# aakhundov/tf-attend-infer-repeat

Measured on AMD Instinct MI355X. Metric: images/sec AIR train step, 50x50 multi-MNIST b=64 N=3, higher is better.
Workload: dtype bf16; 1 GPU; configs[1]: AIR train step, 50x50 canvas, 0-2 objects, batch 64/GPU, 3 steps, 256 LSTM, z=50 (training.py:100-122); global_batch=64, hipgraph=True, steps_per_graph_replay=20, graph_mode=one hipGraph replay = 20 train steps, parallelism=dp1, backward=reference, phase=single order

## Files before the change

tf-attend-infer-repeat_amd/csrc/air_sampler_common.h:

```cpp
#pragma once
#include "air_common.h"
#include <cstdio>
#include <atomic>
#include <type_traits>
#include <cstdlib>
#include <cstring>
#include <cmath>

namespace {

constexpr int THREADS = 256;

struct Tap { float w0, w1; int i0, i1; };

__device__ __forceinline__ Tap axis_tap(int j, int n_out, int n_in, float a, float b, float* t_out = nullptr) {
    const float step = 2.0f / (float)(n_out - 1);
    const float t = (n_out > 1) ? (-1.0f + step * (float)j) : -1.0f;
    const float xs = a * t + b;
    const float X = ((xs + 1.0f) * ((float)n_in - 1.001f)) / 2.0f;
    const float f0 = floorf(X);
    const float lim = (float)(n_in - 1);
    const float c0 = fminf(fmaxf(f0, 0.0f), lim);
    const float c1 = fminf(fmaxf(f0 + 1.0f, 0.0f), lim);
    Tap tp;
// ... 103 lines not shown
        R = R + sh_z[t] * wr;
    }
    return R;
}

__device__ __forceinline__ float compose_clip(float R, float& p1, float& p0) {
    const float r = fmaxf(fminf(R, 1.0f), 0.0f);
    p1 = r + AIR_EPS; p0 = (1.0f - r) + AIR_EPS;
    return r;
}
__device__ __forceinline__ float compose_dloss(float R, float x, float p1, float p0, float gsc) {
    const bool pass = (R <= 1.0f) && (fminf(R, 1.0f) >= 0.0f);
    return pass ? -gsc * (x / p1 - (1.0f - x) / p0) : 0.0f;
}

__device__ __forceinline__ float gauss_kl_term(float plv, float lv, float var, float pv, float mean, float pm) {
    const float d = mean - pm;
    return (((plv - lv) - 1.0f) + var / pv) + (d * d) / pv;
}

struct ComposeLds {
    float* red; float* z; int* act;
    float* kl; float* rec;
    Tap* tx; Tap* ty; float* win;
};
__device__ __forceinline__ ComposeLds compose_lds(float* base, int N, int C, int w) {
    ComposeLds L;
    L.red = base; L.z = base + 16; L.act = reinterpret_cast<int*>(base + 16 + MAX_STEPS);
    L.kl = base + 16 + 2 * MAX_STEPS; L.rec = base + 16 + 3 * MAX_STEPS;
    L.tx = reinterpret_cast<Tap*>(base + 16 + 7 * MAX_STEPS); L.ty = L.tx + (size_t)N * C;
    L.win = reinterpret_cast<float*>(L.ty + (size_t)N * C);
    return L;
}
template <int NWAVES>
__device__ __forceinline__ void compose_vae_kl(const float* ml_all, const float* dyn, int b, int B, int N, int Z, int lane, int wave,
                                               float* sh_kl) {
    for (int t = wave; t < N; t += NWAVES) {
        const float* ml = ml_all + ((size_t)t * B + b) * 2 * Z;
        const float pv = dyn[AIR_DYN_VAE_PV], pm = dyn[AIR_DYN_VAE_PM], plv = dyn[AIR_DYN_VAE_PLV];
        float klt = 0.0f;
        for (int j = lane; j < Z; j += 64) {
            const float lv = ml[Z + j];
            klt += gauss_kl_term(plv, lv, expf(lv), pv, ml[j], pm);
        }
        klt = air_wave_sum(klt);
        if (lane == 0) sh_kl[t] = 0.5f * klt;
    }
}
__device__ __forceinline__ void compose_fetch_records(const float* att, int b, int B, int N, int tid, const ComposeLds& L) {
    if (tid < N) {
        const float* at = att + ((size_t)tid * B + b) * AIR_ATT_STRIDE;
        const float zv = at[AIR_ATT_Z], mk = at[AIR_ATT_MASK], mp = at[AIR_ATT_MASK_PREV];
        const float kz = at[AIR_ATT_KL_Z], ks = at[AIR_ATT_KL_SCALE], kh = at[AIR_ATT_KL_SHIFT];
        L.z[tid] = zv;
        L.act[tid] = mk != 0.0f ? 1 : 0;
        L.rec[4 * tid] = mp; L.rec[4 * tid + 1] = kz; L.rec[4 * tid + 2] = ks; L.rec[4 * tid + 3] = kh;
    }
}
__device__ __forceinline__ void compose_running_loss(const ComposeLds& L, float* att, int b, int B, int N, float& loss, int& digits) {
    loss = 0.0f;
    digits = 0;
    for (int t = 0; t < N; ++t) {
        const bool mask = L.act[t] != 0;
        loss = loss + (L.rec[4 * t] != 0.0f ? L.rec[4 * t + 1] : 0.0f);
        loss = loss + (mask ? L.rec[4 * t + 2] : 0.0f);
        loss = loss + (mask ? L.rec[4 * t + 3] : 0.0f);
        loss = loss + (mask ? L.kl[t] : 0.0f);
        digits += mask ? 1 : 0;
        att[((size_t)t * B + b) * AIR_ATT_STRIDE + AIR_ATT_KL_VAE] = L.kl[t];
    }
}
constexpr int COMPOSE_XPRE = 4;
__device__ __forceinline__ bool compose_prefetch_image(const float* images, size_t base, int CC, int tid, float (&xs)[COMPOSE_XPRE]) {
    const bool xpre = CC <= COMPOSE_XPRE * CF_THREADS;
#pragma unroll
    for (int k = 0; k < COMPOSE_XPRE; ++k) { const int p = tid + k * CF_THREADS; xs[k] = images[base + ((xpre && p < CC) ? p : 0)]; }
    return xpre;
}
template <int OUT, bool G_LDS>
__device__ __forceinline__ float compose_pixels(const ComposeLds& L, const float* images, size_t base, const float (&xs)[COMPOSE_XPRE],
// ... 69 lines not shown
```

tf-attend-infer-repeat_amd/csrc/air_sampler_write_bwd.hip:

```cpp
#include "air_sampler_common.h"

AIR_STAMPS_READER(air_debug_stamps_wb)
#ifdef AIR_STAMPS
static __device__ unsigned long long air_stamps_wg[4096 * 8];
extern "C" int air_debug_stamps_wg(unsigned long long* out, int n) {
    return (int)hipMemcpyFromSymbol(out, HIP_SYMBOL(air_stamps_wg), sizeof(unsigned long long) * (n < 4096 * 8 ? n : 4096 * 8));
}
#define AIR_STAMP_WG(i) do { if (threadIdx.x == 0) air_stamps_wg[((blockIdx.y * gridDim.x + blockIdx.x) & 4095) * 8 + (i)] = wall_clock64(); } while (0)
#define AIR_STAMP_WG_T(i, t) do { if (threadIdx.x == (t)) air_stamps_wg[((blockIdx.y * gridDim.x + blockIdx.x) & 4095) * 8 + (i)] = wall_clock64(); } while (0)
#define AIR_STAMP_WG_ADD(i, t0) do { if (threadIdx.x == 0) air_stamps_wg[((blockIdx.y * gridDim.x + blockIdx.x) & 4095) * 8 + (i)] += wall_clock64() - (t0); } while (0)
#define AIR_STAMP_WG_SET(i, v) do { if (threadIdx.x == 0) air_stamps_wg[((blockIdx.y * gridDim.x + blockIdx.x) & 4095) * 8 + (i)] = (unsigned long long)(v); } while (0)
#define AIR_NOW() wall_clock64()
#else
#define AIR_STAMP_WG(i) do { } while (0)
#define AIR_STAMP_WG_T(i, t) do { } while (0)
#define AIR_STAMP_WG_ADD(i, t0) do { } while (0)
#define AIR_STAMP_WG_SET(i, v) do { } while (0)
#define AIR_NOW() 0ull
#endif

namespace {

typedef __attribute__((address_space(3))) float air_lds_float;
__device__ __forceinline__ void lds_fadd(float* p, float v) {
    asm volatile("ds_add_f32 %0, %1" :: "v"((unsigned)(size_t)(air_lds_float*)p), "v"(v) : "memory");
}

__global__ __launch_bounds__(THREADS) void transformer_bwd_kernel(
    const float* __restrict__ U, const float* __restrict__ theta, const float* __restrict__ d_out,
    float* __restrict__ d_U, float* __restrict__ d_theta, int Hi, int Wi, int Ho, int Wo, int lds_ordered)
{
    extern __shared__ __attribute__((aligned(16))) float smem[];
    const int b = blockIdx.x, tid = threadIdx.x, lane = tid & 63, wave = tid >> 6;
    const int NI = Hi * Wi, NO = Ho * Wo;
    float* sh_red = smem;
    float* sh_th = smem + 32;
    float* sh_U = smem + 40;
    float* sh_dU = sh_U + ((NI + 3) & ~3);
    const float* img = U + (size_t)b * NI;
    const float* g = d_out + (size_t)b * NO;
    if (tid < 6) sh_th[tid] = theta[(size_t)b * 6 + tid];
    for (int p = tid; p < NI; p += THREADS) { sh_U[p] = img[p]; sh_dU[p] = 0.0f; }
    __syncthreads();
    if (d_theta) {
        float s6[6] = {0.f, 0.f, 0.f, 0.f, 0.f, 0.f};
        for (int p = tid; p < NO; p += THREADS) {
            const GenTap t = generic_tap(sh_th, p / Wo, p % Wo, Hi, Wi, Ho, Wo);
            const float Ia = sh_U[t.y0 * Wi + t.x0], Ib = sh_U[t.y1 * Wi + t.x0];
            const float Ic = sh_U[t.y0 * Wi + t.x1], Id = sh_U[t.y1 * Wi + t.x1];
            generic_dtheta_pixel(t, g[p] * Ia, g[p] * Ib, g[p] * Ic, g[p] * Id, Hi, Wi, s6);
        }
// ... 483 lines not shown
template <bool ALLPH>
__device__ __forceinline__ bool wb_open(const air_write_bwd_t& a, WbCtx& k, float& win_pre, float (&g_pre)[8]) {
    if (a.fin_scalars && k.lin == (a.order ? (int)(gridDim.x * gridDim.y) - 1 : 0)) {
        batch_means<WB_THREADS>(a, k.sh_red, k.tid, LoadPlain{});
        __syncthreads();
    }
    AIR_STAMP(40);
    AIR_STAMP_WG(0);
    win_pre = k.tid < k.w * k.w ? k.v[k.tid] : 0.0f;
    if (ALLPH) stage_g_load<WB_THREADS>(k.gsrc, k.CC, k.tid, 0, g_pre);
    if (k.at[AIR_ATT_MASK] == 0.0f) {
        zero_item<WB_THREADS>(k.dgen, k.dgen16, k.dsx, k.w * k.w, k.tid);
        return false;
    }
    wb_item(k, k.at[AIR_ATT_S], k.at[AIR_ATT_X], k.at[AIR_ATT_Y], k.at[AIR_ATT_Z]);
    return true;
}

constexpr int WB_SIG = WB_THREADS - 64;
__device__ __forceinline__ int* fold_last_word(const WbCtx& k) { return reinterpret_cast<int*>(k.sh_red) + (WB_NW - 1) * 8 + 7; }
__device__ __forceinline__ int fold_signal(int32_t* arrive, int tid) {
    int ticket = -1;
    if (tid == WB_SIG) {
        asm volatile("s_waitcnt vmcnt(0)" ::: "memory");
        ticket = __hip_atomic_fetch_add((air_global_int*)arrive, 1, __ATOMIC_RELAXED, __HIP_MEMORY_SCOPE_AGENT);
    }
    return ticket;
}
__device__ __forceinline__ void fold_means(const air_write_bwd_t& a, int32_t* arrive, const WbCtx& k, bool last) {
    if (!last) return;
    batch_means<WB_THREADS>(a, k.sh_red, k.tid, LoadAgent{});
    if (k.tid == 0) store_agent(arrive, 0);
}
__device__ __forceinline__ bool fold_front(const air_write_bwd_t& a, const air_write_fwd_t& f, int32_t* arrive, WbCtx& k, bool owner,
                                           float& win_pre) {
    const int N = a.N, B = a.B, C = k.C, w = k.w, tid = k.tid, b = k.b;
    const ComposeLds L = compose_lds(k.sh_T, N, C, w);
    float* c_sig = L.win + (size_t)N * w * w;
    const size_t base = (size_t)b * k.CC;
    const float mask_own = k.at[AIR_ATT_MASK];
    wb_item(k, k.at[AIR_ATT_S], k.at[AIR_ATT_X], k.at[AIR_ATT_Y], k.at[AIR_ATT_Z]);
    constexpr int WPRE = 4;
    float xs[COMPOSE_XPRE], wpre[WPRE];
    const bool xpre = compose_prefetch_image(f.images, base, k.CC, tid, xs);
#pragma unroll
    for (int q = 0; q < WPRE; ++q) {
        const int it = tid + q * WB_THREADS;
        wpre[q] = compose_window_at(a.vrec, b, B, w, it < N * w * w ? it : 0);
    }
    if (owner) compose_vae_kl<WB_NW>(f.ml, f.dyn, b, B, N, f.Z, k.lane, k.wave, L.kl);
    compose_stage_taps(a.att, b, B, N, C, w, tid, WB_THREADS, L.tx, L.ty);
#pragma unroll
    for (int q = 0; q < WPRE; ++q) { const int it = tid + q * WB_THREADS; if (it < N * w * w) L.win[it] = wpre[q]; }
    compose_stage_windows(a.vrec, b, B, N, w, tid + WPRE * WB_THREADS, WB_THREADS, L.win);
    compose_fetch_records(a.att, b, B, N, tid, L);
    __syncthreads();
    if (!owner && mask_own == 0.0f) {
        zero_item<WB_THREADS>(k.dgen, k.dgen16, k.dsx, w * w, tid);
        return false;
    }
    if (owner && tid == 0) {
        float loss;
        int digits;
        compose_running_loss(L, f.att, b, B, N, loss, digits);
        f.run_loss[b] = loss;
        c_sig[0] = loss;
        c_sig[1] = __builtin_bit_cast(float, digits);
    }
    float acc = compose_pixels<2, true>(L, f.images, base, xs, xpre, N, C, w, f.dyn[AIR_DYN_GRAD_SCALE], tid, owner,
                                        f.recon, f.d_recon, k.sh_g);
    if (owner) {
        acc = air_block_sum_n<WB_NW>(acc, L.red);
        const float rl = -acc;
        if (tid == 0) f.rec_loss[b] = rl;
        if (tid == WB_SIG) {
            store_agent(f.loss_item + b, c_sig[0] + rl);
            store_agent(f.run_digits + b, __builtin_bit_cast(int, c_sig[1]));
        }
    }
    AIR_STAMP_WG(7);
    if (mask_own == 0.0f) {
        zero_item<WB_THREADS>(k.dgen, k.dgen16, k.dsx, w * w, tid);
        const int ticket = fold_signal(arrive, tid);
        int* sh_last = fold_last_word(k);
        if (tid == WB_SIG) *sh_last = ticket == a.B - 1 ? 1 : 0;
        __syncthreads();
        fold_means(a, arrive, k, *sh_last != 0);
        return false;
    }
    win_pre = tid < w * w ? L.win[(size_t)k.t * w * w + tid] : 0.0f;
    return true;
}

template <bool ALLPH, int PH0, int PH1>
__device__ __forceinline__ void stage_terms(const WbCtx& k) {
    const int C = k.C, di = WB_THREADS / C, dj = WB_THREADS % C;
    int i = k.tid / C, j = k.tid % C;
    for (int p = k.tid; p < k.CC; p += WB_THREADS) {
        const Tap tx = k.sh_tx[j], ty = k.sh_ty[i];
        const float gp = k.z * (ALLPH ? k.sh_g[p] : k.gsrc[p]);
        const int4 ci = k.sh_ci[j], ri = k.sh_ri[i];
#pragma unroll
        for (int ph = PH0; ph < PH1; ++ph)
            k.sh_T[(ALLPH ? ph * k.CCp : 0) + wb_term_pos(ci, ri, i, j, C, ph)] = wb_tap_weight(tx, ty, ph) * gp;
        i += di; j += dj;
        if (j >= C) { j -= C; ++i; }
    }
}
template <bool ALLPH, int PH0, int PH1, bool THETA>
__device__ __forceinline__ void carried_terms(const WbCtx& k, WbGrad& G) {
    const int C = k.C, w = k.w;
    const int RPP = WB_THREADS / C, bj = k.tid % C, bi0 = k.tid / C;
    if (bi0 >= RPP) return;
// ... 318 lines not shown
}
template <bool ALLPH>
__device__ __forceinline__ bool carried_slot_short(const WbCtx& k, const WbSlot& s) {
    bool short_s = true;
    if (s.is_slot) {
#pragma unroll
        for (int ph = 0; ph < 4; ++ph) { int st, n; slot_run<ALLPH>(k, ph, s.sp, s.sq, st, n); short_s = short_s && n <= WB_CHUNK_MIN; }
    }
    return short_s;
}
template <bool ALLPH, int PH0, int PH1>
__device__ __forceinline__ void carried_slot(const WbCtx& k, const WbSlot& s, float& P_s, float& corr_s, float& Q_s, bool short_s, bool& have_s,
                                             float& acc) {
    if (!s.is_slot) return;
#pragma unroll
    for (int ph = PH0; ph < PH1; ++ph) {
        int start, n;
        slot_run<ALLPH>(k, ph, s.sp, s.sq, start, n);
        n = max(n, 0);
        if (short_s) { acc = stream_add(acc, k.sh_T, start, n); continue; }
        const int cs = wb_chunk_len(n);
        for (int k0 = 0; k0 < n; k0 += cs) {
            if (have_s) corr_s += Q_s - P_s;
            float c = 0.0f, q = P_s;
            stream_add2(c, q, k.sh_T, start + k0, min(cs, n - k0));
            Q_s = q;
            P_s += c;
            have_s = true;
        }
        acc = Q_s + corr_s;
    }
}

template <bool FOLD>
__device__ __forceinline__ void write_bwd_graph_allph_body(const air_write_bwd_t& a, int seq_flags, const air_write_fwd_t* fp,
                                                           int32_t* arrive) {
    extern __shared__ __attribute__((aligned(16))) float smem[];
    const bool lds_ordered = seq_flags & 1, ring_ok = seq_flags & 2;
    WbCtx k = wb_ctx<true>(a, smem);
    const bool owner = FOLD && k.t == 0;
    float win_pre = 0.0f, g_pre[8];
    if constexpr (FOLD) {
        AIR_STAMP(40);
        AIR_STAMP_WG(0);
        if (!fold_front(a, *fp, arrive, k, owner, win_pre)) return;
    } else if (!wb_open<true>(a, k, win_pre, g_pre)) return;
    wb_setup<!FOLD>(k, win_pre, g_pre);
    const WbSlot s = wb_slot<false>(k, lds_ordered, ring_ok);
    WbGrad G = {0.f, 0.f, 0.f, 0.f, 0.f};
    float acc = 0.0f, theta_g[THETA_G];
    AIR_STAMP_WG(1);
    stage_terms<true, 0, 4>(k);
    __syncthreads();
    AIR_STAMP(43);
    AIR_STAMP_WG(2);
    chains<true>(k, s, 0, 4, acc);
    AIR_STAMP(49);
    publish(k, s, acc);
    if (FOLD) theta_take(k, WB_TH0, WB_THN, theta_g);
    AIR_STAMP(39);
    __syncthreads();
    AIR_STAMP(44);
    AIR_STAMP_WG(3);
    if (k.wave < 4) corner_accumulate<true>(k, k.wave, 0, 4, lds_ordered, ring_ok);
    else {
        const int ticket = owner ? fold_signal(arrive, k.tid) : -1;
        theta_loop<FOLD>(k, WB_TH0, WB_THN, theta_g, G);
        if (owner && k.tid == WB_SIG) *fold_last_word(k) = ticket == a.B - 1 ? 1 : 0;
    }
    AIR_STAMP(48);
    AIR_STAMP_WG(4);
    __syncthreads();
    AIR_STAMP_WG(5);
    graph_tail(k, s);
    if (owner) fold_means(a, arrive, k, *fold_last_word(k) != 0);
    AIR_STAMP(47);
    AIR_STAMP_WG(6);
}

__device__ __forceinline__ void write_bwd_graph_onetap_body(const air_write_bwd_t& a, int seq_flags) {
    extern __shared__ __attribute__((aligned(16))) float smem[];
    const bool lds_ordered = seq_flags & 1, ring_ok = seq_flags & 2;
    WbCtx k = wb_ctx<false>(a, smem);
    float win_pre = 0.0f, g_pre[8];
    if (!wb_open<false>(a, k, win_pre, g_pre)) return;
    wb_setup<false>(k, win_pre, g_pre);
    const WbSlot s = wb_slot<false>(k, lds_ordered, ring_ok);
    WbGrad G = {0.f, 0.f, 0.f, 0.f, 0.f};
    float acc = 0.0f, theta_g[THETA_G];
    AIR_STAMP_WG_SET(1, 0); AIR_STAMP_WG_SET(2, 0); AIR_STAMP_WG_SET(3, 0);
    AIR_STAMP_WG_SET(4, (__builtin_amdgcn_s_getreg(20 | (0 << 6) | (3 << 11)) << 16) | __builtin_amdgcn_s_getreg(4 | (0 << 6) | (15 << 11)));
    AIR_STAMP_WG_SET(5, (lds_ordered ? 0xf : 0) | (k.sh_cn[0] + k.sh_cn[1] + k.sh_cn[2] + k.sh_cn[3]) << 4);
    for (int ph = 0; ph < 4; ++ph) {
        const unsigned long long ta = AIR_NOW();
        if (ph == 0) stage_terms<false, 0, 1>(k);
        else if (ph == 1) stage_terms<false, 1, 2>(k);
        else if (ph == 2) stage_terms<false, 2, 3>(k);
        else stage_terms<false, 3, 4>(k);
        __syncthreads();
        AIR_STAMP(50 + 3 * ph);
        AIR_STAMP_WG_ADD(1, ta);
        const unsigned long long tb = AIR_NOW();
        chains<false>(k, s, ph, ph + 1, acc);
        __syncthreads();
// ... 300 lines not shown
```

tf-attend-infer-repeat_amd/csrc/air_wgrad.hip:

```cpp
#include "air_common.h"
#include "air_mfma.h"
#include <type_traits>
#include <cstring>
#include <cstdlib>

namespace airw {

using airm::f32x4; using airm::bf16x8;
using airm::zero_acc; using airm::read_tr_bf16x8; using airm::aligned16; using airm::aligned8;

constexpr int THREADS = 256;
constexpr int BT = 64;
constexpr int KC = 32;
constexpr int LS = BT + 16;
constexpr int KB = 64;
constexpr int NIMG_W = 3;
constexpr int MAXP = AIR_MAX_WGRAD_PROBLEMS;

struct Prob {
    const float* A; const float* dY; float* dW; float* db;
    const unsigned short* A16; const unsigned short* dY16;
    int M, N, K, lda, ldb, ldc;
    int head_pack, Hs, Hh, Hz;
    int tiles_n, first_block;
// ... 46 lines not shown
}

__device__ __forceinline__ void mfma_2x2(f32x4 (&acc)[2][2], const bf16x8 (&av)[2], const bf16x8 (&bv)[2]) {
#pragma unroll
    for (int i = 0; i < 2; ++i)
#pragma unroll
        for (int j = 0; j < 2; ++j)
            acc[i][j] = __builtin_amdgcn_mfma_f32_16x16x32_bf16(av[i], bv[j], acc[i][j], 0, 0, 0);
}

__device__ __forceinline__ void sum_kruns(float (&csum)[4]) {
#pragma unroll
    for (int j = 0; j < 4; ++j) {
        float s = csum[j];
        s += __shfl_xor(s, 1); s += __shfl_xor(s, 2); s += __shfl_xor(s, 4);
        csum[j] = s;
    }
}
__device__ __forceinline__ float store_db(float* db, const float (&v)[4], int c0, int lim) {
    float sq = 0.0f;
#pragma unroll
    for (int j = 0; j < 4; ++j)
        if (c0 + j < lim) { db[c0 + j] = v[j]; sq += v[j] * v[j]; }
    return sq;
}

__device__ __forceinline__ void publish_sq(float sq, float* sq_partials, int32_t* istate, int part, float* sq_red) {
    sq = air_block_sum_256(sq, sq_red);
    if (threadIdx.x == 0) {
        sq_partials[part] = sq;
        if (part == 0 && istate) istate[AIR_IST_GLOBAL_STEP] += 1;
    }
}

__device__ __forceinline__ float store_tile(const Prob& pr, int m0, int n0, const float* Ct, float sq)
{
    const int tid = threadIdx.x;
    const int M = pr.M, N = pr.N, ldc = pr.ldc;
    float* dW = pr.dW;
    if (!pr.head_pack) {
        const bool vecC = ((ldc & 3) == 0) && aligned16(dW);
#pragma unroll
        for (int r = 0; r < 4; ++r) {
            const int row = (tid >> 4) + 16 * r, col = (tid & 15) * 4;
            const int m = m0 + row, n = n0 + col;
            if (m >= M) continue;
            const float4 t = *reinterpret_cast<const float4*>(&Ct[row * LS + col]);
            float* dst = dW + (size_t)m * ldc + n;
            if (vecC && n + 3 < N) { if (dW) *reinterpret_cast<float4*>(dst) = t; sq += (t.x * t.x + t.y * t.y) + (t.z * t.z + t.w * t.w); }
            else {
                if (n < N) { if (dW) dst[0] = t.x; sq += t.x * t.x; }
                if (n + 1 < N) { if (dW) dst[1] = t.y; sq += t.y * t.y; }
                if (n + 2 < N) { if (dW) dst[2] = t.z; sq += t.z * t.z; }
                if (n + 3 < N) { if (dW) dst[3] = t.w; sq += t.w * t.w; }
            }
        }
    } else {
        const int Hs = pr.Hs, Hh = pr.Hh, Hz = pr.Hz;
        for (int it = tid; it < 7 * BT; it += THREADS) {
            const int o = it / BT, col = it % BT, n = n0 + col;
            const int hd = air_out_head(o);
            const int off = air_head_off(Hs, Hh, hd);
            const int wd = air_head_wid(Hs, Hh, Hz, hd);
            if (m0 == 0 && n < N && n >= off && n < off + wd) {
                const float t = Ct[o * LS + col];
                dW[(size_t)o * ldc + (n - off)] = t;
// ... 267 lines not shown
__device__ __forceinline__ float bias_tw(const Prob& pr, int n0)
{
    const int tid = threadIdx.x;
    const int N = pr.N, K = pr.K, ldb = pr.ldb;
    const int bg = tid & 7, bq = (tid & 127) >> 3;
    const bool bias_thread = tid >= 128;
    float csum[4] = {0.f, 0.f, 0.f, 0.f};
    if (bias_thread) {
        const bool vec = ((ldb & 3) == 0) && aligned16(pr.dY);
        const int nimg = (K + KB - 1) / KB;
        float4 cur[8], nxt[8];
        auto fetch_img = [&](float4 (&v)[8], int c) __attribute__((always_inline)) {
#pragma unroll
            for (int r = 0; r < 8; ++r)
                v[r] = vec ? fetch4<true>(pr.dY, ldb, c * KB + bg * 8 + r, n0 + 4 * bq, K, N)
                           : fetch4<false>(pr.dY, ldb, c * KB + bg * 8 + r, n0 + 4 * bq, K, N);
        };
        fetch_img(cur, 0);
        for (int c = 0; c < nimg; ++c) {
            if (c + 1 < nimg) fetch_img(nxt, c + 1);
#pragma unroll
            for (int r = 0; r < 8; ++r) {
                const float4 t = mask4(cur[r], c * KB + bg * 8 + r, n0 + 4 * bq, K, N);
                csum[0] += t.x; csum[1] += t.y; csum[2] += t.z; csum[3] += t.w;
            }
#pragma unroll
            for (int r = 0; r < 8; ++r) cur[r] = nxt[r];
        }
    }
    sum_kruns(csum);
    return (bias_thread && bg == 0) ? store_db(pr.db, csum, n0 + 4 * bq, N) : 0.0f;
}

constexpr int T8 = NIMG_W * KB * 16 / THREADS;
__device__ __forceinline__ void issue_pieces(uint2 (&r)[T8], const char* base, bool w16, int kr, int c0, int K, int cols, int ld) {
    const int tid = threadIdx.x;
    if (w16) {
#pragma unroll
        for (int i = 0; i < T8 / 2; ++i) {
            const int t = tid + THREADS * i, k = kr + (t >> 3), col = c0 + (t & 7) * 8;
            const bool ok = k < K && col < cols;
            const uint4 x = *reinterpret_cast<const uint4*>(base + (ok ? ((unsigned)k * (unsigned)ld + (unsigned)col) * 2u : 0u));
            r[2 * i] = ok ? make_uint2(x.x, x.y) : make_uint2(0u, 0u);
            r[2 * i + 1] = ok ? make_uint2(x.z, x.w) : make_uint2(0u, 0u);
        }
    } else {
#pragma unroll
        for (int i = 0; i < T8; ++i) {
            const int t = tid + THREADS * i, k = kr + (t >> 4), col = c0 + (t & 15) * 4;
            const bool ok = k < K && col < cols;
            const uint2 x = *reinterpret_cast<const uint2*>(base + (ok ? ((unsigned)k * (unsigned)ld + (unsigned)col) * 2u : 0u));
            r[i] = ok ? x : make_uint2(0u, 0u);
        }
    }
}
__device__ __forceinline__ void store_pieces(const uint2 (&r)[T8], unsigned short* img, bool w16) {
    const int tid = threadIdx.x;
    if (w16) {
#pragma unroll
        for (int i = 0; i < T8 / 2; ++i)
            *reinterpret_cast<uint4*>(&img[(tid + THREADS * i) * 8]) = make_uint4(r[2 * i].x, r[2 * i].y, r[2 * i + 1].x, r[2 * i + 1].y);
    } else {
#pragma unroll
        for (int i = 0; i < T8; ++i) *reinterpret_cast<uint2*>(&img[(tid + THREADS * i) * 4]) = r[i];
    }
}

__device__ __forceinline__ float tile_bf16_tw(const Prob& pr, int m0, int n0, unsigned short* Img)
{
    constexpr int NIMG = NIMG_W;
    const int tid = threadIdx.x, lane = tid & 63, wave = tid >> 6;
    const int wm = (wave >> 1) * 32, wn = (wave & 1) * 32;
    const int M = pr.M, N = pr.N, K = pr.K, lda = pr.lda, ldb = pr.ldb;
    const char* Ab = reinterpret_cast<const char*>(pr.A16);
    const char* Yb = reinterpret_cast<const char*>(pr.dY16);
    unsigned short* ImgA = Img;
    unsigned short* ImgB = Img + NIMG * KB * BT;
    const bool a16 = rows16(pr.A16, lda) && (M & 7) == 0;
    const bool b16 = rows16(pr.dY16, ldb) && (N & 7) == 0;
    const bool bias_block = (pr.db != nullptr) && owns_bias(pr, m0, n0);

    f32x4 acc[2][2];
    zero_acc(acc);

    uint2 ra[T8], rb[T8];
    auto issue_round = [&](int kr) __attribute__((always_inline)) {
        issue_pieces(ra, Ab, a16, kr, m0, K, M, lda);
        issue_pieces(rb, Yb, b16, kr, n0, K, N, ldb);
    };
    AIR_STAMP(1);
    issue_round(0);
    AIR_STAMP(2);
    for (int kr = 0; kr < K; kr += NIMG * KB) {
        if (kr > 0) __syncthreads();
        store_pieces(ra, ImgA, a16);
        store_pieces(rb, ImgB, b16);
        AIR_STAMP(3);
        if (kr + NIMG * KB < K) issue_round(kr + NIMG * KB);
        __syncthreads();
        AIR_STAMP(4);
        const int il = lane & 15;
#pragma unroll
        for (int c = 0; c < NIMG; ++c)
            if (kr + c * KB < K) {
#pragma unroll
                for (int ks = 0; ks < 2; ++ks) {
                    const int krow = c * KB + ks * 32 + (lane >> 4) * 8 + (il >> 2);
                    const unsigned short* pa = &ImgA[krow * BT + wm + (il & 3) * 4];
                    const unsigned short* pb = &ImgB[krow * BT + wn + (il & 3) * 4];
                    bf16x8 av[2], bv[2];
#pragma unroll
                    for (int i = 0; i < 2; ++i) av[i] = read_tr_bf16x8(pa + i * 16, BT);
#pragma unroll
                    for (int j = 0; j < 2; ++j) bv[j] = read_tr_bf16x8(pb + j * 16, BT);
                    mfma_2x2(acc, av, bv);
                }
            }
    }
    AIR_STAMP(5);
    const float sq = bias_block ? bias_tw(pr, n0) : 0.0f;
    __syncthreads();
    acc_to_lds(acc, reinterpret_cast<float*>(Img), wm, wn, lane);
    __syncthreads();
    return sq;
}

typedef unsigned u32x4 __attribute__((ext_vector_type(4)));
typedef unsigned u32x2 __attribute__((ext_vector_type(2)));

constexpr int STRIP_KMAX = 256;
#ifdef AIR_STAMPS
#ifndef STRIP_STAMP_BLOCK
#define STRIP_STAMP_BLOCK 600
#endif
#define STRIP_STAMP(i) do { if (blockIdx.x == STRIP_STAMP_BLOCK && threadIdx.x == 0) air_stamps_dev[i] = wall_clock64(); } while (0)
#else
#define STRIP_STAMP(i) do { } while (0)
#endif
constexpr int STRIP_LDS = STRIP_KMAX * BT * 2;
constexpr int STRIP_MAXG = 16;
constexpr int STRIP_TAIL = (4 + STRIP_MAXG * 16) * 4;
template <int NPER,
          bool A8>
__device__ __forceinline__ void run_strip_bf16(const Prob& pr, int m0, int n0, unsigned short* Img, float* __restrict__ sq_partials,
                                               int32_t* __restrict__ istate, float* sq_red)
{
    const int tid = threadIdx.x, lane = tid & 63, wave = tid >> 6;
    const int wm = (wave >> 1) * 32, wn = (wave & 1) * 32;
    const int G = pr.strip;
    const unsigned lda = (unsigned)pr.lda, ldb = (unsigned)pr.ldb;
    const char* Ab = reinterpret_cast<const char*>(pr.A16);
    const char* Yb = reinterpret_cast<const char*>(pr.dY16);
    unsigned short* ImgB = Img;
    const bool has_bias = pr.db != nullptr;

    float* bias_park = sq_red + 4;
    if (has_bias) {
        for (int j = 0; j < G; ++j) {
            if (!owns_bias(pr, m0, n0 + j * BT)) continue;
            const float b = bias_tw(pr, n0 + j * BT);
            if (tid >= 128 && (tid & 7) == 0) bias_park[j * 16 + ((tid & 127) >> 3)] = b;
        }
        __syncthreads();
    }

    STRIP_STAMP(0);
    const unsigned k0 = (unsigned)(tid >> 3), c8 = (unsigned)(tid & 7) * 8u;
    auto issue_b = [&](u32x4 (&rb)[NPER], int nn) __attribute__((always_inline)) {
#pragma unroll
        for (int i = 0; i < NPER; ++i)
            rb[i] = *reinterpret_cast<const u32x4*>(Yb + ((k0 + 32u * i) * ldb + (unsigned)nn + c8) * 2u);
    };
    auto stage_b = [&](const u32x4 (&rb)[NPER]) __attribute__((always_inline)) {
#pragma unroll
        for (int i = 0; i < NPER; ++i)
            *reinterpret_cast<u32x4*>(&ImgB[(tid + THREADS * i) * 8]) = rb[i];
    };
    const int mb = m0 / BT;
    const int rot = (mb + (mb >> 3)) % G;
    auto tile_at = [&](int j) { int t = j + rot; if (t >= G) t -= G; return t; };
    const int il = lane & 15;
    bf16x8 av[NPER][2];
    {
        u32x4 rb[NPER];
        if constexpr (!A8) {
            u32x4 ra[NPER];
#pragma unroll
            for (int i = 0; i < NPER; ++i)
                ra[i] = *reinterpret_cast<const u32x4*>(Ab + ((k0 + 32u * i) * lda + (unsigned)m0 + c8) * 2u);
// ... 26 lines not shown
        stage_b(rb);
    }
    STRIP_STAMP(1);

    const int part0 = pr.first_part + mb * pr.tiles_n + n0 / BT;
    for (int j = 0; j < G; ++j) {
        const int tj = tile_at(j);
        const int nj = n0 + tj * BT;
        __syncthreads();
        STRIP_STAMP(2 + 6 * j);
        u32x4 rb[NPER];
        issue_b(rb, n0 + tile_at(j + 1 < G ? j + 1 : j) * BT);
        __builtin_amdgcn_sched_barrier(0);
        f32x4 acc[2][2];
        zero_acc(acc);
#pragma unroll
        for (int kk = 0; kk < NPER; ++kk) {
            const int krow = kk * 32 + (lane >> 4) * 8 + (il >> 2);
            const unsigned short* pb = &ImgB[krow * BT + wn + (il & 3) * 4];
            bf16x8 bv[2];
#pragma unroll
            for (int jj = 0; jj < 2; ++jj) bv[jj] = read_tr_bf16x8(pb + jj * 16, BT);
            mfma_2x2(acc, av[kk], bv);
        }
        STRIP_STAMP(3 + 6 * j);
        const float bias_sq = (has_bias && owns_bias(pr, m0, nj) && tid >= 128 && (tid & 7) == 0) ? bias_park[tj * 16 + ((tid & 127) >> 3)] : 0.0f;
        __syncthreads();
        float* Ct = reinterpret_cast<float*>(ImgB);
        acc_to_lds(acc, Ct, wm, wn, lane);
        __syncthreads();
        STRIP_STAMP(4 + 6 * j);
        const float sq = store_tile(pr, m0, nj, Ct, bias_sq);
        STRIP_STAMP(5 + 6 * j);
        if (sq_partials) publish_sq(sq, sq_partials, istate, part0 + tj, sq_red);
        STRIP_STAMP(6 + 6 * j);
        if (j + 1 < G) {
            __syncthreads();
            stage_b(rb);
        }
        STRIP_STAMP(7 + 6 * j);
    }
}
template <bool A8>
__device__ __forceinline__ void run_strip_k(const Prob& pr, int m0, int n0, unsigned short* Img, float* __restrict__ sq_partials,
                                            int32_t* __restrict__ istate, float* sq_red)
{
    if (pr.K == 256) run_strip_bf16<8, A8>(pr, m0, n0, Img, sq_partials, istate, sq_red);
    else if (pr.K == 192) run_strip_bf16<6, A8>(pr, m0, n0, Img, sq_partials, istate, sq_red);
    else if (pr.K == 128) run_strip_bf16<4, A8>(pr, m0, n0, Img, sq_partials, istate, sq_red);
    else run_strip_bf16<2, A8>(pr, m0, n0, Img, sq_partials, istate, sq_red);
}

__device__ __forceinline__ void run_bias_wg(const Prob& pr, int n0, int part, float* __restrict__ sq_partials, float* sq_red)
{
    const int tid = threadIdx.x;
    const int N = pr.N, K = pr.K;
    const unsigned ldb = (unsigned)pr.ldb;
    const float* __restrict__ Y = pr.dY;
    const int g = tid & 7, q = (tid >> 3) & 15, h = tid >> 7;
    const int col = n0 + 4 * q;
    const bool vec = ((ldb & 3u) == 0u) && aligned16(Y);
    const int nimg = (K + KB - 1) / KB;
    float csum[4] = {0.f, 0.f, 0.f, 0.f};
    auto fetch_img = [&](f32x4 (&v)[8], int c) __attribute__((always_inline)) {
        if (c >= nimg) c = nimg - 1;
#pragma unroll
        for (int r = 0; r < 8; ++r) {
            const int row = c * KB + g * 8 + r;
            const bool okr = row < K;
            const unsigned at = (unsigned)row * ldb + (unsigned)col;
            if (vec) v[r] = *reinterpret_cast<const f32x4*>(Y + ((okr && col < N) ? at : 0u));
            else {
                v[r].x = Y[(okr && col < N) ? at : 0u];
// ... 48 lines not shown
    for (int i = 0; i < MAXP; ++i)
        if (i < tab.count && tab.p[i].bias_first >= 0 && block >= tab.p[i].bias_first) k = i;
    const Prob& pb = tab.p[k];
    const int idx = block - pb.bias_first;
    run_bias_wg(pb, idx * BT, pb.bias_part + idx, sq_partials, sq_red);
}

#ifdef AIR_STAMPS
static __device__ unsigned long long air_wgrad_wg_stamps[2048 * 4];
#define WG_STAMP(b, i, v) do { if (threadIdx.x == 0 && (b) < 2048) air_wgrad_wg_stamps[(b) * 4 + (i)] = (unsigned long long)(v); } while (0)
#define WG_HWID() ((__builtin_amdgcn_s_getreg(20 | (0 << 6) | (3 << 11)) << 16) | __builtin_amdgcn_s_getreg(4 | (0 << 6) | (15 << 11)))
#else
#define WG_STAMP(b, i, v) do { } while (0)
#define WG_HWID() 0
#endif

__device__ __forceinline__ void run_tile_bf16(const Table& tab, int block, unsigned short* Img, float* __restrict__ sq_partials,
                                              int32_t* __restrict__ istate, float* sq_red)
{
    if (block < tab.nbias) { run_bias_block(tab, block, sq_partials, sq_red); return; }
    int m0, n0;
    const Prob& pr = find_tile(tab, block, m0, n0);
    WG_STAMP(block, 3, pr.K * 16 + pr.strip);
    AIR_STAMP(0);
    if (pr.strip > 0) {
        if (rows16(pr.A16, pr.lda) && (pr.M % BT) == 0) run_strip_k<false>(pr, m0, n0, Img, sq_partials, istate, sq_red);
        else run_strip_k<true>(pr, m0, n0, Img, sq_partials, istate, sq_red);
        return;
    }
    const float bias_sq = twin_ok(pr) ? tile_bf16_tw(pr, m0, n0, Img) : tile_bf16(pr, m0, n0, Img);
    AIR_STAMP(6);
    const float sq = store_tile(pr, m0, n0, reinterpret_cast<const float*>(Img), bias_sq);
    AIR_STAMP(7);
    if (sq_partials) publish_sq(sq, sq_partials, istate, pr.first_part + (block - pr.first_block), sq_red);
    AIR_STAMP(8);
}

}

using namespace airw;

namespace {

__global__ __launch_bounds__(THREADS) void wgrad_grouped_kernel(Table tab, float* __restrict__ sq_partials, int32_t* __restrict__ istate)
{
    __shared__ __attribute__((aligned(16))) float As[2][KC * LS];
    __shared__ __attribute__((aligned(16))) float Bs[2][KC * LS];
    const int block = (int)blockIdx.x;
    __shared__ float sq_red[4 + 64];
    if (block < tab.nbias) { run_bias_block(tab, block, sq_partials, sq_red); return; }
    int m0, n0;
    const Prob& pr = find_tile(tab, block, m0, n0);
    const float bias_sq = tile_f32<6>(pr, m0, n0, As, Bs);
    const float sq = store_tile(pr, m0, n0, &As[0][0], 0.0f) + bias_sq;
    if (sq_partials) publish_sq(sq, sq_partials, istate, pr.first_part + (block - pr.first_block), sq_red);
}


__global__ __launch_bounds__(THREADS) __attribute__((amdgpu_waves_per_eu(3, 3))) void wgrad_grouped_bf16_kernel(
    Table tab, float* __restrict__ sq_partials, int32_t* __restrict__ istate)
{
    extern __shared__ __attribute__((aligned(16))) unsigned short Img[];
    float* sq_red = reinterpret_cast<float*>(Img + 2 * NIMG_W * BT * KB);
    const int block = (int)blockIdx.x;
    WG_STAMP(block, 0, wall_clock64());
    WG_STAMP(block, 2, WG_HWID());
    run_tile_bf16(tab, block, Img, sq_partials, istate, sq_red);
// ... 99 lines not shown
```

Baseline: 380,500 images/sec.

## Elect cheapest step as fold owner and overlap chains with corner accumulation

The fold owner is no longer always step 0. Each wave estimates the corner-term cost of one step from its taps, and the active step with the fewest corner terms becomes the owner that does the compose/KL/loss work. The VAE KL is split into a prefetch and a later sum so its loads overlap the pixel compose, and the running-loss computation moves into the signalling thread. When corner work is heavy and LDS ordering is on, waves 0-3 run corner accumulation before their chains instead of after, with the reversed corner index, which removes one block barrier. The cost is extra tap and ballot work in the front end and a more complex ownership and scheduling scheme.

```diff
diff --git a/tf-attend-infer-repeat_amd/csrc/air_sampler_common.h b/tf-attend-infer-repeat_amd/csrc/air_sampler_common.h
--- a/tf-attend-infer-repeat_amd/csrc/air_sampler_common.h
+++ b/tf-attend-infer-repeat_amd/csrc/air_sampler_common.h
@@ -159,20 +159,40 @@
     L.win = reinterpret_cast<float*>(L.ty + (size_t)N * C);
     return L;
 }
+struct KlPre { float lv, mean, pv, pm, plv; };
+__device__ __forceinline__ KlPre compose_vae_kl_prefetch(const float* ml_all, const float* dyn, int b, int B, int N, int Z, int lane, int wave) {
+    KlPre p = {0.0f, 0.0f, 0.0f, 0.0f, 0.0f};
+    if (wave < N) {
+        p.pv = dyn[AIR_DYN_VAE_PV]; p.pm = dyn[AIR_DYN_VAE_PM]; p.plv = dyn[AIR_DYN_VAE_PLV];
+        if (lane < Z) {
+            const float* ml = ml_all + ((size_t)wave * B + b) * 2 * Z;
+            p.lv = ml[Z + lane]; p.mean = ml[lane];
+        }
+    }
+    return p;
+}
+template <int NWAVES, bool PRE>
+__device__ __forceinline__ void compose_vae_kl_sum(const KlPre& pre, const float* ml_all, const float* dyn, int b, int B, int N, int Z,
+                                                   int lane, int wave, float* sh_kl) {
+    for (int t = wave; t < N; t += NWAVES) {
+        const float* ml = ml_all + ((size_t)t * B + b) * 2 * Z;
+        const float pv = PRE ? pre.pv : dyn[AIR_DYN_VAE_PV], pm = PRE ? pre.pm : dyn[AIR_DYN_VAE_PM];
+        const float plv = PRE ? pre.plv : dyn[AIR_DYN_VAE_PLV];
+        float klt = 0.0f;
+        for (int j = lane; j < Z; j += 64) {
+            const bool first = PRE && t == wave && j == lane;
+            const float lv = first ? pre.lv : ml[Z + j];
+            const float mean = first ? pre.mean : ml[j];
+            klt += gauss_kl_term(plv, lv, expf(lv), pv, mean, pm);
+        }
+        klt = air_wave_sum(klt);
+        if (lane == 0) sh_kl[t] = 0.5f * klt;
+    }
+}
 template <int NWAVES>
 __device__ __forceinline__ void compose_vae_kl(const float* ml_all, const float* dyn, int b, int B, int N, int Z, int lane, int wave,
                                                float* sh_kl) {
-    for (int t = wave; t < N; t += NWAVES) {
-        const float* ml = ml_all + ((size_t)t * B + b) * 2 * Z;
-        const float pv = dyn[AIR_DYN_VAE_PV], pm = dyn[AIR_DYN_VAE_PM], plv = dyn[AIR_DYN_VAE_PLV];
-        float klt = 0.0f;
-        for (int j = lane; j < Z; j += 64) {
-            const float lv = ml[Z + j];
-            klt += gauss_kl_term(plv, lv, expf(lv), pv, ml[j], pm);
-        }
-        klt = air_wave_sum(klt);
-        if (lane == 0) sh_kl[t] = 0.5f * klt;
-    }
+    compose_vae_kl_sum<NWAVES, false>(KlPre{}, ml_all, dyn, b, B, N, Z, lane, wave, sh_kl);
 }
 __device__ __forceinline__ void compose_fetch_records(const float* att, int b, int B, int N, int tid, const ComposeLds& L) {
     if (tid < N) {
diff --git a/tf-attend-infer-repeat_amd/csrc/air_sampler_write_bwd.hip b/tf-attend-infer-repeat_amd/csrc/air_sampler_write_bwd.hip
--- a/tf-attend-infer-repeat_amd/csrc/air_sampler_write_bwd.hip
+++ b/tf-attend-infer-repeat_amd/csrc/air_sampler_write_bwd.hip
@@ -11,12 +11,20 @@
 #define AIR_STAMP_WG_ADD(i, t0) do { if (threadIdx.x == 0) air_stamps_wg[((blockIdx.y * gridDim.x + blockIdx.x) & 4095) * 8 + (i)] += wall_clock64() - (t0); } while (0)
 #define AIR_STAMP_WG_SET(i, v) do { if (threadIdx.x == 0) air_stamps_wg[((blockIdx.y * gridDim.x + blockIdx.x) & 4095) * 8 + (i)] = (unsigned long long)(v); } while (0)
 #define AIR_NOW() wall_clock64()
+static __device__ unsigned long long air_stamps_wg2[4096 * 8];
+extern "C" int air_debug_stamps_wg2(unsigned long long* out, int n) {
+    return (int)hipMemcpyFromSymbol(out, HIP_SYMBOL(air_stamps_wg2), sizeof(unsigned long long) * (n < 4096 * 8 ? n : 4096 * 8));
+}
+#define AIR_STAMP_WG2_SET(i, v) do { if (threadIdx.x == 0) air_stamps_wg2[((blockIdx.y * gridDim.x + blockIdx.x) & 4095) * 8 + (i)] = (unsigned long long)(v); } while (0)
+#define AIR_STAMP_WG2_LAST(i) atomicMax(&air_stamps_wg2[((blockIdx.y * gridDim.x + blockIdx.x) & 4095) * 8 + (i)], (unsigned long long)wall_clock64())
 #else
 #define AIR_STAMP_WG(i) do { } while (0)
 #define AIR_STAMP_WG_T(i, t) do { } while (0)
 #define AIR_STAMP_WG_ADD(i, t0) do { } while (0)
 #define AIR_STAMP_WG_SET(i, v) do { } while (0)
 #define AIR_NOW() 0ull
+#define AIR_STAMP_WG2_SET(i, v) do { } while (0)
+#define AIR_STAMP_WG2_LAST(i) do { } while (0)
 #endif
 
 namespace {
@@ -566,14 +574,31 @@
     batch_means<WB_THREADS>(a, k.sh_red, k.tid, LoadAgent{});
     if (k.tid == 0) store_agent(arrive, 0);
 }
-__device__ __forceinline__ bool fold_front(const air_write_bwd_t& a, const air_write_fwd_t& f, int32_t* arrive, WbCtx& k, bool owner,
+__device__ __forceinline__ int fold_corner_terms(float s, float x, float y, int C, int w, int lane) {
+    const float ia = 1.0f / s, bx = (-x) / s, by = (-y) / s;
+    int cols = 0, rows = 0;
+    for (int j0 = 0; j0 < C; j0 += 64) {
+        const int j = j0 + lane;
+        const bool in = j < C;
+        const Tap tx = axis_tap(min(j, C - 1), C, w, ia, bx), ty = axis_tap(min(j, C - 1), C, w, ia, by);
+        cols += __popcll(__ballot(in && tx.i0 == 0)) + __popcll(__ballot(in && tx.i0 == w - 1)) +
+                __popcll(__ballot(in && tx.i1 == 0)) + __popcll(__ballot(in && tx.i1 == w - 1));
+        rows += __popcll(__ballot(in && ty.i0 == 0)) + __popcll(__ballot(in && ty.i0 == w - 1)) +
+                __popcll(__ballot(in && ty.i1 == 0)) + __popcll(__ballot(in && ty.i1 == w - 1));
+    }
+    return cols * rows;
+}
+__device__ __forceinline__ bool fold_front(const air_write_bwd_t& a, const air_write_fwd_t& f, int32_t* arrive, WbCtx& k, bool& owner,
                                            float& win_pre) {
     const int N = a.N, B = a.B, C = k.C, w = k.w, tid = k.tid, b = k.b;
     const ComposeLds L = compose_lds(k.sh_T, N, C, w);
-    float* c_sig = L.win + (size_t)N * w * w;
+    int* const sh_cost = reinterpret_cast<int*>(L.red);
     const size_t base = (size_t)b * k.CC;
     const float mask_own = k.at[AIR_ATT_MASK];
     wb_item(k, k.at[AIR_ATT_S], k.at[AIR_ATT_X], k.at[AIR_ATT_Y], k.at[AIR_ATT_Z]);
+    static_assert(WB_NW >= MAX_STEPS, "one wave per step counts the election's costs");
+    const float* eat = a.att + ((size_t)min(k.wave, N - 1) * B + b) * AIR_ATT_STRIDE;
+    const float e_s = eat[AIR_ATT_S], e_x = eat[AIR_ATT_X], e_y = eat[AIR_ATT_Y], e_mask = eat[AIR_ATT_MASK];
     constexpr int WPRE = 4;
     float xs[COMPOSE_XPRE], wpre[WPRE];
     const bool xpre = compose_prefetch_image(f.images, base, k.CC, tid, xs);
@@ -582,37 +607,43 @@
         const int it = tid + q * WB_THREADS;
         wpre[q] = compose_window_at(a.vrec, b, B, w, it < N * w * w ? it : 0);
     }
-    if (owner) compose_vae_kl<WB_NW>(f.ml, f.dyn, b, B, N, f.Z, k.lane, k.wave, L.kl);
     compose_stage_taps(a.att, b, B, N, C, w, tid, WB_THREADS, L.tx, L.ty);
+    if (k.wave < N) {
+        const int terms = fold_corner_terms(e_s, e_x, e_y, C, w, k.lane);
+        if (k.lane == 0) sh_cost[k.wave] = e_mask != 0.0f ? terms : INT32_MAX;
+    }
 #pragma unroll
     for (int q = 0; q < WPRE; ++q) { const int it = tid + q * WB_THREADS; if (it < N * w * w) L.win[it] = wpre[q]; }
     compose_stage_windows(a.vrec, b, B, N, w, tid + WPRE * WB_THREADS, WB_THREADS, L.win);
     compose_fetch_records(a.att, b, B, N, tid, L);
     __syncthreads();
+    int own = 0, best = INT32_MAX;
+    for (int t = 0; t < N; ++t) { const int c = sh_cost[t]; if (c < best) { best = c; own = t; } }
+    owner = own == k.t;
     if (!owner && mask_own == 0.0f) {
         zero_item<WB_THREADS>(k.dgen, k.dgen16, k.dsx, w * w, tid);
         return false;
     }
-    if (owner && tid == 0) {
-        float loss;
-        int digits;
-        compose_running_loss(L, f.att, b, B, N, loss, digits);
-        f.run_loss[b] = loss;
-        c_sig[0] = loss;
-        c_sig[1] = __builtin_bit_cast(float, digits);
-    }
+    KlPre kl_pre = {0.0f, 0.0f, 0.0f, 0.0f, 0.0f};
+    if (owner) kl_pre = compose_vae_kl_prefetch(f.ml, f.dyn, b, B, N, f.Z, k.lane, k.wave);
     float acc = compose_pixels<2, true>(L, f.images, base, xs, xpre, N, C, w, f.dyn[AIR_DYN_GRAD_SCALE], tid, owner,
                                         f.recon, f.d_recon, k.sh_g);
     if (owner) {
+        compose_vae_kl_sum<WB_NW, true>(kl_pre, f.ml, f.dyn, b, B, N, f.Z, k.lane, k.wave, L.kl);
         acc = air_block_sum_n<WB_NW>(acc, L.red);
         const float rl = -acc;
         if (tid == 0) f.rec_loss[b] = rl;
         if (tid == WB_SIG) {
-            store_agent(f.loss_item + b, c_sig[0] + rl);
-            store_agent(f.run_digits + b, __builtin_bit_cast(int, c_sig[1]));
+            float loss;
+            int digits;
+            compose_running_loss(L, f.att, b, B, N, loss, digits);
+            f.run_loss[b] = loss;
+            store_agent(f.loss_item + b, loss + rl);
+            store_agent(f.run_digits + b, digits);
         }
     }
     AIR_STAMP_WG(7);
+    AIR_STAMP_WG2_SET(0, owner ? 1 : 0);
     if (mask_own == 0.0f) {
         zero_item<WB_THREADS>(k.dgen, k.dgen16, k.dsx, w * w, tid);
         const int ticket = fold_signal(arrive, tid);
@@ -997,13 +1028,17 @@
     }
 }
 
+#ifndef AIR_WB_BESIDE_MIN
+#define AIR_WB_BESIDE_MIN 676
+#endif
+constexpr int WB_BESIDE_MIN = AIR_WB_BESIDE_MIN;
 template <bool FOLD>
 __device__ __forceinline__ void write_bwd_graph_allph_body(const air_write_bwd_t& a, int seq_flags, const air_write_fwd_t* fp,
                                                            int32_t* arrive) {
     extern __shared__ __attribute__((aligned(16))) float smem[];
     const bool lds_ordered = seq_flags & 1, ring_ok = seq_flags & 2;
     WbCtx k = wb_ctx<true>(a, smem);
-    const bool owner = FOLD && k.t == 0;
+    bool owner = false;
     float win_pre = 0.0f, g_pre[8];
     if constexpr (FOLD) {
         AIR_STAMP(40);
@@ -1014,27 +1049,43 @@
     const WbSlot s = wb_slot<false>(k, lds_ordered, ring_ok);
     WbGrad G = {0.f, 0.f, 0.f, 0.f, 0.f};
     float acc = 0.0f, theta_g[THETA_G];
+    const int corner_terms = (k.sh_cn[0] + k.sh_cn[1]) + (k.sh_cn[2] + k.sh_cn[3]);
+    const bool beside = lds_ordered && corner_terms >= WB_BESIDE_MIN;
     AIR_STAMP_WG(1);
+    AIR_STAMP_WG2_SET(1, corner_terms); AIR_STAMP_WG2_SET(2, beside ? 1 : 0); AIR_STAMP_WG2_SET(3, 0); AIR_STAMP_WG2_SET(4, 0);
+    AIR_STAMP_WG2_SET(5, k.sh_cn[beside ? 3 : 0]);
     stage_terms<true, 0, 4>(k);
+    if (FOLD && beside) theta_take(k, WB_TH0, WB_THN, theta_g);
     __syncthreads();
     AIR_STAMP(43);
     AIR_STAMP_WG(2);
-    chains<true>(k, s, 0, 4, acc);
-    AIR_STAMP(49);
-    publish(k, s, acc);
-    if (FOLD) theta_take(k, WB_TH0, WB_THN, theta_g);
-    AIR_STAMP(39);
-    __syncthreads();
+    if (!beside || k.wave >= 4) {
+        chains<true>(k, s, 0, 4, acc);
+        AIR_STAMP(49);
+        publish(k, s, acc);
+        if (beside) AIR_STAMP_WG2_LAST(3);
+    }
+    if (!beside) {
+        if (FOLD) theta_take(k, WB_TH0, WB_THN, theta_g);
+        AIR_STAMP(39);
+        __syncthreads();
+    }
     AIR_STAMP(44);
     AIR_STAMP_WG(3);
-    if (k.wave < 4) corner_accumulate<true>(k, k.wave, 0, 4, lds_ordered, ring_ok);
-    else {
+    if (k.wave < 4) {
+        corner_accumulate<true>(k, beside ? 3 - k.wave : k.wave, 0, 4, lds_ordered, ring_ok);
+        AIR_STAMP(48);
+        AIR_STAMP_WG(4);
+        if (beside) {
+            chains<true>(k, s, 0, 4, acc);
+            publish(k, s, acc);
+            AIR_STAMP_WG2_LAST(4);
+        }
+    } else {
         const int ticket = owner ? fold_signal(arrive, k.tid) : -1;
         theta_loop<FOLD>(k, WB_TH0, WB_THN, theta_g, G);
         if (owner && k.tid == WB_SIG) *fold_last_word(k) = ticket == a.B - 1 ? 1 : 0;
     }
-    AIR_STAMP(48);
-    AIR_STAMP_WG(4);
     __syncthreads();
     AIR_STAMP_WG(5);
     graph_tail(k, s);
```

Result: no change. 383,000 images/sec, median of 6 (+0.7%).

## Overlap bias reduction with wgrad MFMA and defer per-tile sq publishing in strips

Applied to the files above, without the earlier changes.

In the twin-image wgrad tile path, when K fits in a single round, bias-column loads and sums run on the upper waves and overlap the A/B staging and MFMA loop, instead of a separate bias pass afterwards. In strip mode, each tile's squared-norm partial is reduced within a wave and parked in LDS. All tile partials are then published once at the end, which removes a block-wide reduction barrier per tile. The single-tile path also switches to the parked wave-sum publish. This adds register pressure from the float4 bias buffers and enlarges the shared tail.

```diff
diff --git a/tf-attend-infer-repeat_amd/csrc/air_wgrad.hip b/tf-attend-infer-repeat_amd/csrc/air_wgrad.hip
--- a/tf-attend-infer-repeat_amd/csrc/air_wgrad.hip
+++ b/tf-attend-infer-repeat_amd/csrc/air_wgrad.hip
@@ -102,6 +102,14 @@
         if (part == 0 && istate) istate[AIR_IST_GLOBAL_STEP] += 1;
     }
 }
+__device__ __forceinline__ void park_sq(float sq, float* red) {
+    sq = air_wave_sum(sq);
+    if ((threadIdx.x & 63) == 0) red[threadIdx.x >> 6] = sq;
+}
+__device__ __forceinline__ void publish_parked(const float* red, float* sq_partials, int32_t* istate, int part) {
+    sq_partials[part] = ((red[0] + red[1]) + red[2]) + red[3];
+    if (part == 0 && istate) istate[AIR_IST_GLOBAL_STEP] += 1;
+}
 
 __device__ __forceinline__ float store_tile(const Prob& pr, int m0, int n0, const float* Ct, float sq)
 {
@@ -435,6 +443,25 @@
     return (bias_thread && bg == 0) ? store_db(pr.db, csum, n0 + 4 * bq, N) : 0.0f;
 }
 
+__device__ __forceinline__ bool bias_early(const Prob& pr) {
+    return pr.K <= NIMG_W * KB && (pr.K % KB) == 0 && ((pr.ldb & 3) == 0) && aligned16(pr.dY);
+}
+__device__ __forceinline__ void bias_issue(float4 (&v)[8], const Prob& pr, int n0, int c) {
+    const int bg = threadIdx.x & 7, col = n0 + ((threadIdx.x & 127) >> 3) * 4;
+    const float* p = pr.dY + ((size_t)(unsigned)(c * KB + bg * 8) * (unsigned)pr.ldb + (unsigned)(col < pr.N ? col : 0));
+    const size_t step = (size_t)(unsigned)pr.ldb;
+#pragma unroll
+    for (int r = 0; r < 8; ++r) v[r] = *reinterpret_cast<const float4*>(p + r * step);
+}
+__device__ __forceinline__ void bias_add(float (&csum)[4], const float4 (&v)[8], const Prob& pr, int n0, int c) {
+    const int bg = threadIdx.x & 7, bq = (threadIdx.x & 127) >> 3;
+#pragma unroll
+    for (int r = 0; r < 8; ++r) {
+        const float4 t = mask4(v[r], c * KB + bg * 8 + r, n0 + 4 * bq, pr.K, pr.N);
+        csum[0] += t.x; csum[1] += t.y; csum[2] += t.z; csum[3] += t.w;
+    }
+}
+
 constexpr int T8 = NIMG_W * KB * 16 / THREADS;
 __device__ __forceinline__ void issue_pieces(uint2 (&r)[T8], const char* base, bool w16, int kr, int c0, int K, int cols, int ld) {
     const int tid = threadIdx.x;
@@ -486,22 +513,11 @@
     f32x4 acc[2][2];
     zero_acc(acc);
 
-    uint2 ra[T8], rb[T8];
-    auto issue_round = [&](int kr) __attribute__((always_inline)) {
+    auto issue_round = [&](uint2 (&ra)[T8], uint2 (&rb)[T8], int kr) __attribute__((always_inline)) {
         issue_pieces(ra, Ab, a16, kr, m0, K, M, lda);
         issue_pieces(rb, Yb, b16, kr, n0, K, N, ldb);
     };
-    AIR_STAMP(1);
-    issue_round(0);
-    AIR_STAMP(2);
-    for (int kr = 0; kr < K; kr += NIMG * KB) {
-        if (kr > 0) __syncthreads();
-        store_pieces(ra, ImgA, a16);
-        store_pieces(rb, ImgB, b16);
-        AIR_STAMP(3);
-        if (kr + NIMG * KB < K) issue_round(kr + NIMG * KB);
-        __syncthreads();
-        AIR_STAMP(4);
+    auto multiply = [&](int kr) __attribute__((always_inline)) {
         const int il = lane & 15;
 #pragma unroll
         for (int c = 0; c < NIMG; ++c)
@@ -519,9 +535,52 @@
                     mfma_2x2(acc, av, bv);
                 }
             }
-    }
-    AIR_STAMP(5);
-    const float sq = bias_block ? bias_tw(pr, n0) : 0.0f;
+    };
+    float sq = 0.0f;
+    const bool early = bias_block && bias_early(pr);
+    AIR_STAMP(1);
+    if (K <= NIMG * KB) {
+        const bool bias_wave = early && tid >= 128;
+        uint2 ra[T8], rb[T8];
+        float4 b0[8], b1[8];
+        float csum[4] = {0.f, 0.f, 0.f, 0.f};
+        issue_round(ra, rb, 0);
+        if (bias_wave) bias_issue(b0, pr, n0, 0);
+        AIR_STAMP(2);
+        store_pieces(ra, ImgA, a16);
+        store_pieces(rb, ImgB, b16);
+        if (bias_wave) {
+            bias_add(csum, b0, pr, n0, 0);
+            if (K > KB) bias_issue(b1, pr, n0, 1);
+            if (K > 2 * KB) bias_issue(b0, pr, n0, 2);
+        }
+        __builtin_amdgcn_sched_barrier(0);
+        AIR_STAMP(3);
+        __syncthreads();
+        AIR_STAMP(4);
+        multiply(0);
+        AIR_STAMP(5);
+        if (early) {
+            if (bias_wave) {
+                if (K > KB) bias_add(csum, b1, pr, n0, 1);
+                if (K > 2 * KB) bias_add(csum, b0, pr, n0, 2);
+            }
+            sum_kruns(csum);
+            if (bias_wave && (tid & 7) == 0) sq = store_db(pr.db, csum, n0 + ((tid & 127) >> 3) * 4, N);
+        }
+    } else {
+        uint2 ra[T8], rb[T8];
+        issue_round(ra, rb, 0);
+        for (int kr = 0; kr < K; kr += NIMG * KB) {
+            if (kr > 0) __syncthreads();
+            store_pieces(ra, ImgA, a16);
+            store_pieces(rb, ImgB, b16);
+            if (kr + NIMG * KB < K) issue_round(ra, rb, kr + NIMG * KB);
+            __syncthreads();
+            multiply(kr);
+        }
+    }
+    if (bias_block && !early) sq = bias_tw(pr, n0);
     __syncthreads();
     acc_to_lds(acc, reinterpret_cast<float*>(Img), wm, wn, lane);
     __syncthreads();
@@ -542,7 +601,7 @@
 #endif
 constexpr int STRIP_LDS = STRIP_KMAX * BT * 2;
 constexpr int STRIP_MAXG = 16;
-constexpr int STRIP_TAIL = (4 + STRIP_MAXG * 16) * 4;
+constexpr int STRIP_TAIL = (4 + STRIP_MAXG * 16 + STRIP_MAXG * 4) * 4;
 template <int NPER,
           bool A8>
 __device__ __forceinline__ void run_strip_bf16(const Prob& pr, int m0, int n0, unsigned short* Img, float* __restrict__ sq_partials,
@@ -558,6 +617,7 @@
     const bool has_bias = pr.db != nullptr;
 
     float* bias_park = sq_red + 4;
+    float* tile_park = bias_park + STRIP_MAXG * 16;
     if (has_bias) {
         for (int j = 0; j < G; ++j) {
             if (!owns_bias(pr, m0, n0 + j * BT)) continue;
@@ -650,13 +710,17 @@
         STRIP_STAMP(4 + 6 * j);
         const float sq = store_tile(pr, m0, nj, Ct, bias_sq);
         STRIP_STAMP(5 + 6 * j);
-        if (sq_partials) publish_sq(sq, sq_partials, istate, part0 + tj, sq_red);
+        if (sq_partials) park_sq(sq, tile_park + 4 * tj);
         STRIP_STAMP(6 + 6 * j);
         if (j + 1 < G) {
             __syncthreads();
             stage_b(rb);
         }
         STRIP_STAMP(7 + 6 * j);
+    }
+    if (sq_partials) {
+        __syncthreads();
+        if (tid < G) publish_parked(tile_park + 4 * tid, sq_partials, istate, part0 + tid);
     }
 }
 template <bool A8>
@@ -771,7 +835,11 @@
     AIR_STAMP(6);
     const float sq = store_tile(pr, m0, n0, reinterpret_cast<const float*>(Img), bias_sq);
     AIR_STAMP(7);
-    if (sq_partials) publish_sq(sq, sq_partials, istate, pr.first_part + (block - pr.first_block), sq_red);
+    if (sq_partials) {
+        park_sq(sq, sq_red);
+        __syncthreads();
+        if (threadIdx.x == 0) publish_parked(sq_red, sq_partials, istate, pr.first_part + (block - pr.first_block));
+    }
     AIR_STAMP(8);
 }
 
```

After: 380,200 images/sec before, 385,300 images/sec after (median of 6 runs). +1.3%, better.
